# amazon-science/instruct-video-to-video

Measured on AMD Instinct MI355X. Metric: denoised video-frames/sec (16f@256x384, 50 DDIM steps), higher is better.
Workload: dtype fp16; 1 GPU; C2: 1 clip/step = VAE-encode + 50 DDIM steps (3-way CFG, text 7.5 / video 1.5) + VAE-decode, 16 frames @ 256x384, random-init full-width UNet+VAE; 5 independent clips in flight per GPU (stacked into every UNet launch, B = 3 x clips); frames=16, height=256, width=384, ddim_steps=50, clips_per_gpu=5, parallelism=clip-parallel x1, one all_gather, hip_graph=True, cfg_branch_streams=False, concurrent_clips=5, clip_mode=stacked, driver_mode=False, full=False

## Files before the change

### instruct-video-to-video_amd/csrc/winograd.hip

```cpp
#include "common.h"

namespace {

template <bool UP> __device__ __forceinline__ int lds_px(int sp) { return UP ? sp : sp ^ ((sp >> 1) & 1); }

template <bool NORM, bool UP>
__global__ __launch_bounds__(256) void wino_input_kernel(const half_t* __restrict__ x, const half_t* __restrict__ x2, const float* __restrict__ ab,
                                                         half_t* __restrict__ V, int64_t ldx, int64_t ldx2, int C1, int C, int NB, int H, int W,
                                                         int ipb, int images_per_sample, int silu, int64_t group_rows, int band_tr) {
    extern __shared__ __attribute__((aligned(16))) char smem[];
    const int tid = threadIdx.x, chunk = tid & 7, item0 = tid >> 3;
    const int nb0 = (int)blockIdx.x * ipb, c0 = (int)blockIdx.y * 64;
    const int trows = UP ? H : (H + 1) >> 1;
    const int tr0 = (int)blockIdx.z * band_tr, tr1 = min(tr0 + band_tr, trows);
    const bool whole = band_tr >= trows;
    const int row0 = whole ? 0 : (UP ? tr0 - 1 : 2 * tr0 - 1);
    const int nrows = whole ? H : (UP ? (tr1 - tr0) + 2 : 2 * (tr1 - tr0) + 2);
    const int HW = H * W, SW = nrows * W;
    const int SWs = UP ? SW : (SW + 1) & ~1;
    const bool second = x2 != nullptr && c0 >= C1;
    const half_t* src = second ? x2 + (c0 - C1) + chunk * 8 : x + c0 + chunk * 8;
    const int64_t ld = second ? ldx2 : ldx;
    const int nimg = min(ipb, NB - nb0);
    for (int it = item0; it < nimg * SW; it += 32) {
        const int img = it / SW, sp = it - img * SW;
        const int iy = row0 + sp / W;
        if ((unsigned)iy >= (unsigned)H) continue;
        half8 v = *(const half8*)(src + ((int64_t)(nb0 + img) * HW + sp + row0 * W) * ld);
        if (NORM) {
            const float* p = ab + ((int64_t)((nb0 + img) / images_per_sample) * C + c0 + chunk * 8) * 2;
            const float4 p0 = *(const float4*)p, p1 = *(const float4*)(p + 4), p2 = *(const float4*)(p + 8), p3 = *(const float4*)(p + 12);
            const float sc[8] = {p0.x, p0.z, p1.x, p1.z, p2.x, p2.z, p3.x, p3.z}, sh[8] = {p0.y, p0.w, p1.y, p1.w, p2.y, p2.w, p3.y, p3.w};
#pragma unroll
            for (int e = 0; e < 8; ++e) {
                float f = fmaf((float)v[e], sc[e], sh[e]);
                if (silu) f = silu_f(f);
                v[e] = (half_t)f;
            }
        }
        *(half8*)(smem + ((int64_t)img * SWs + lds_px<UP>(sp)) * 128 + chunk * 16) = v;
    }
    __syncthreads();
    if constexpr (UP) {
        const int bt = (tr1 - tr0) * W;
        for (int it = item0; it < nimg * bt; it += 32) {
            const int img = it / bt, tb_ = it - img * bt;
            const int y = tr0 + tb_ / W, xx = tb_ - (tb_ / W) * W;
            const int t = y * W + xx;
            const char* base = smem + (int64_t)img * SWs * 128 + chunk * 16;
            float hz[3][3][8];
#pragma unroll
            for (int r = 0; r < 3; ++r) {
                const int iy = y - 1 + r;
                float d[3][8];
#pragma unroll
                for (int c = 0; c < 3; ++c) {
                    const int ix = xx - 1 + c;
                    const bool ok = (unsigned)iy < (unsigned)H && (unsigned)ix < (unsigned)W;
                    half8 v = {0, 0, 0, 0, 0, 0, 0, 0};
                    if (ok) v = *(const half8*)(base + lds_px<UP>((iy - row0) * W + ix) * 128);
#pragma unroll
                    for (int e = 0; e < 8; ++e) d[c][e] = (float)v[e];
                }
#pragma unroll
                for (int e = 0; e < 8; ++e) {
                    hz[r][0][e] = d[0][e] - d[1][e];
                    hz[r][1][e] = 2.f * d[1][e];
                    hz[r][2][e] = d[1][e] - d[2][e];
                }
            }
            const int64_t trow = (int64_t)(nb0 + img) * HW + t;
            half_t* dst = V + trow * C + c0 + chunk * 8;
#pragma unroll
            for (int j = 0; j < 3; ++j) {
                half8 o[3];
#pragma unroll
                for (int e = 0; e < 8; ++e) {
                    o[0][e] = (half_t)(hz[0][j][e] - hz[1][j][e]);
                    o[1][e] = (half_t)(2.f * hz[1][j][e]);
                    o[2][e] = (half_t)(hz[1][j][e] - hz[2][j][e]);
                }
#pragma unroll
                for (int i = 0; i < 3; ++i) *(half8*)(dst + (int64_t)(i * 3 + j) * group_rows * C) = o[i];
            }
        }
        return;
    }
    const int th = (H + 1) >> 1, tw = (W + 1) >> 1, ntile = th * tw;
    const int bt = (tr1 - tr0) * tw;
    for (int it = item0; it < nimg * bt; it += 32) {
        const int img = it / bt, tb_ = it - img * bt;
        const int ty = tr0 + tb_ / tw, tx = tb_ - (tb_ / tw) * tw;
        const int t = ty * tw + tx;
        const char* base = smem + (int64_t)img * SWs * 128 + chunk * 16;
        float hz[4][4][8];
#pragma unroll
        for (int r = 0; r < 4; ++r) {
            const int iy = 2 * ty - 1 + r;
            float d[4][8];
#pragma unroll
            for (int c = 0; c < 4; ++c) {
                const int ix = 2 * tx - 1 + c;
                const bool ok = (unsigned)iy < (unsigned)H && (unsigned)ix < (unsigned)W;
                half8 v = {0, 0, 0, 0, 0, 0, 0, 0};
                if (ok) v = *(const half8*)(base + lds_px<UP>((iy - row0) * W + ix) * 128);
#pragma unroll
                for (int e = 0; e < 8; ++e) d[c][e] = (float)v[e];
            }
#pragma unroll
            for (int e = 0; e < 8; ++e) {
                hz[r][0][e] = d[0][e] - d[2][e];
                hz[r][1][e] = d[1][e] + d[2][e];
                hz[r][2][e] = d[2][e] - d[1][e];
                hz[r][3][e] = d[1][e] - d[3][e];
            }
        }
        const int64_t trow = (int64_t)(nb0 + img) * ntile + t;
        half_t* dst = V + trow * C + c0 + chunk * 8;
#pragma unroll
        for (int j = 0; j < 4; ++j) {
            half8 o[4];
#pragma unroll
            for (int e = 0; e < 8; ++e) {
                o[0][e] = (half_t)(hz[0][j][e] - hz[2][j][e]);
                o[1][e] = (half_t)(hz[1][j][e] + hz[2][j][e]);
                o[2][e] = (half_t)(hz[2][j][e] - hz[1][j][e]);
                o[3][e] = (half_t)(hz[1][j][e] - hz[3][j][e]);
            }
#pragma unroll
            for (int i = 0; i < 4; ++i) *(half8*)(dst + (int64_t)(i * 4 + j) * group_rows * C) = o[i];
        }
    }
}

template <bool RES, bool RB, bool UP>
__global__ __launch_bounds__(256) void wino_output_kernel(const half_t* __restrict__ Mo, const float* __restrict__ bias, const float* __restrict__ row_bias,
                                                          const half_t* __restrict__ res, half_t* __restrict__ y, int64_t group_rows, int64_t ntiles_total,
                                                          int Cout, int H, int W, int64_t ld_rb, int rows_per_group, int64_t ldr, int64_t ldy) {
    const int c8 = Cout >> 3;
    const int64_t idx = (int64_t)blockIdx.x * 256 + threadIdx.x;
    const int64_t tile = idx / c8;
    if (tile >= ntiles_total) return;
    const int ch = (int)(idx - tile * c8) * 8;
    const int th = UP ? H : (H + 1) >> 1, tw = UP ? W : (W + 1) >> 1, ntile = th * tw;
    const int OW = UP ? 2 * W : W, OH = UP ? 2 * H : H;
    const int nb = (int)(tile / ntile), t = (int)(tile - (int64_t)nb * ntile);
    const int ty = t / tw, tx = t - ty * tw;
    const half_t* src = Mo + tile * Cout + ch;
    float s[2][4][8];
    if constexpr (UP) {
#pragma unroll
        for (int j = 0; j < 3; ++j) {
            half8 m[3];
#pragma unroll
            for (int i = 0; i < 3; ++i) m[i] = *(const half8*)(src + (int64_t)(i * 3 + j) * group_rows * Cout);
            const int jj = j == 2 ? 3 : j;
#pragma unroll
            for (int e = 0; e < 8; ++e) {
                s[0][jj][e] = (float)m[0][e] + (float)m[1][e];
                s[1][jj][e] = (float)m[1][e] - (float)m[2][e];
            }
        }
#pragma unroll
        for (int e = 0; e < 8; ++e) s[0][2][e] = s[1][2][e] = 0.f;
    } else {
#pragma unroll
        for (int j = 0; j < 4; ++j) {
            half8 m[4];
#pragma unroll
            for (int i = 0; i < 4; ++i) m[i] = *(const half8*)(src + (int64_t)(i * 4 + j) * group_rows * Cout);
#pragma unroll
            for (int e = 0; e < 8; ++e) {
                s[0][j][e] = (float)m[0][e] + (float)m[1][e] + (float)m[2][e];
                s[1][j][e] = (float)m[1][e] - (float)m[2][e] - (float)m[3][e];
            }
        }
    }
    float b[8];
    {
        const float4 b0 = bias ? *(const float4*)(bias + ch) : make_float4(0.f, 0.f, 0.f, 0.f), b1 = bias ? *(const float4*)(bias + ch + 4) : make_float4(0.f, 0.f, 0.f, 0.f);
        b[0] = b0.x; b[1] = b0.y; b[2] = b0.z; b[3] = b0.w; b[4] = b1.x; b[5] = b1.y; b[6] = b1.z; b[7] = b1.w;
    }
    const int64_t m00 = ((int64_t)nb * OH + 2 * ty) * OW + 2 * tx;
    if (RB) {
        const float* rb = row_bias + (m00 / rows_per_group) * ld_rb + ch;
        const float4 r0 = *(const float4*)rb, r1 = *(const float4*)(rb + 4);
        b[0] += r0.x; b[1] += r0.y; b[2] += r0.z; b[3] += r0.w; b[4] += r1.x; b[5] += r1.y; b[6] += r1.z; b[7] += r1.w;
    }
#pragma unroll
    for (int i = 0; i < 2; ++i)
#pragma unroll
        for (int jj = 0; jj < 2; ++jj) {
            if (!UP && (2 * ty + i >= OH || 2 * tx + jj >= OW)) continue;
            const int64_t m = m00 + (int64_t)i * OW + jj;
            float v[8];
#pragma unroll
            for (int e = 0; e < 8; ++e)
                v[e] = (jj == 0 ? s[i][0][e] + s[i][1][e] + s[i][2][e] : s[i][1][e] - s[i][2][e] - s[i][3][e]) + b[e];
            if (RES) {
                const half8 r = *(const half8*)(res + m * ldr + ch);
#pragma unroll
                for (int e = 0; e < 8; ++e) v[e] += (float)r[e];
            }
            half8 o;
#pragma unroll
            for (int e = 0; e < 8; ++e) o[e] = (half_t)v[e];
            *(half8*)(y + m * ldy + ch) = o;
        }
}

}

extern "C" int insv2v_winograd_input(const insv2v_winograd_in_desc* dp, insv2v_stream_t stream) {
    if (!dp) return INSV2V_EINVAL;
    const insv2v_winograd_in_desc& d = *dp;
    if (!d.x || !d.v || d.NB <= 0 || d.H <= 0 || d.W <= 0 || d.C <= 0) return INSV2V_EINVAL;
    if ((d.C % 64) || (d.x2 && (d.C1 <= 0 || d.C1 >= d.C || (d.C1 % 64)))) return INSV2V_EUNSUPPORTED;
    if ((d.ldx & 7) || ((uintptr_t)d.x & 15) || ((uintptr_t)d.v & 15) || (d.x2 && ((d.ldx2 & 7) || ((uintptr_t)d.x2 & 15)))) return INSV2V_EINVAL;
    if (d.gn_ab && (d.gn_images_per_sample <= 0 || ((uintptr_t)d.gn_ab & 15))) return INSV2V_EINVAL;
    const int HW = d.H * d.W, ntile = d.upsample ? HW : ((d.H + 1) / 2) * ((d.W + 1) / 2);
    const int HWs = d.upsample ? HW : (HW + 1) & ~1;
    const int64_t tiles = (int64_t)d.NB * ntile;
    if (d.v_group_rows < tiles) return INSV2V_EINVAL;
    const int trows = d.upsample ? d.H : (d.H + 1) / 2;
    int band_tr = trows, ipb = 1;
    if (HWs * 128 <= 64 * 1024) {
        ipb = 32 / ntile;
        if (ipb < 1) ipb = 1;
        while (ipb > 1 && ipb * HWs * 128 > 64 * 1024) --ipb;
    } else {
        const int max_rows = 64 * 1024 / (d.W * 128);
        band_tr = d.upsample ? max_rows - 2 : (max_rows - 2) / 2;
        if (band_tr < 1) return INSV2V_EUNSUPPORTED;
    }
    const int nbands = (trows + band_tr - 1) / band_tr;
    const int srows = nbands == 1 ? d.H : (d.upsample ? band_tr + 2 : 2 * band_tr + 2);
    const dim3 grid((unsigned)((d.NB + ipb - 1) / ipb), (unsigned)(d.C / 64), (unsigned)nbands);
    const int slots = srows * d.W;
    const size_t lds = (size_t)ipb * (d.upsample ? slots : (slots + 1) & ~1) * 128;
#define WINO_IN(NORM, UP)                                                                                                                             \
    hipLaunchKernelGGL((wino_input_kernel<NORM, UP>), grid, dim3(256), lds, as_stream(stream), (const half_t*)d.x, (const half_t*)d.x2, d.gn_ab, (half_t*)d.v, \
                       d.ldx, d.ldx2, d.x2 ? d.C1 : d.C, d.C, d.NB, d.H, d.W, ipb, d.gn_ab ? d.gn_images_per_sample : 1, d.gn_ab ? d.gn_silu : 0, d.v_group_rows, band_tr)
    if (d.gn_ab) { if (d.upsample) WINO_IN(true, true); else WINO_IN(true, false); }
    else { if (d.upsample) WINO_IN(false, true); else WINO_IN(false, false); }
#undef WINO_IN
    return launch_status();
}

extern "C" int insv2v_winograd_output(const insv2v_winograd_out_desc* dp, insv2v_stream_t stream) {
    if (!dp) return INSV2V_EINVAL;
    const insv2v_winograd_out_desc& d = *dp;
    if (!d.m || !d.y || d.NB <= 0 || d.H <= 0 || d.W <= 0 || d.Cout <= 0) return INSV2V_EINVAL;
    if (d.Cout & 7) return INSV2V_EUNSUPPORTED;
    if ((d.ldy & 7) || ((uintptr_t)d.m & 15) || ((uintptr_t)d.y & 15) || (d.residual && ((d.ldr & 7) || ((uintptr_t)d.residual & 15)))) return INSV2V_EINVAL;
    if ((d.bias && ((uintptr_t)d.bias & 15)) || (d.row_bias && (((uintptr_t)d.row_bias & 15) || (d.ld_rb & 3) || d.rows_per_group <= 0 || d.rows_per_group % (d.H * d.W * (d.upsample ? 4 : 1)))))
        return INSV2V_EINVAL;
    const int64_t tiles = d.upsample ? (int64_t)d.NB * d.H * d.W : (int64_t)d.NB * ((d.H + 1) / 2) * ((d.W + 1) / 2);
    if (d.m_group_rows < tiles) return INSV2V_EINVAL;
    const int64_t n = tiles * (d.Cout / 8);
    const dim3 grid((unsigned)((n + 255) / 256));
#define WINO_OUT(RES, RB, UP)                                                                                                                        \
    hipLaunchKernelGGL((wino_output_kernel<RES, RB, UP>), grid, dim3(256), 0, as_stream(stream), (const half_t*)d.m, d.bias, d.row_bias, (const half_t*)d.residual, \
                       (half_t*)d.y, d.m_group_rows, tiles, d.Cout, d.H, d.W, d.ld_rb, d.rows_per_group, d.ldr, d.ldy)
    if (d.upsample) {
        if (d.residual) { if (d.row_bias) WINO_OUT(true, true, true); else WINO_OUT(true, false, true); }
        else { if (d.row_bias) WINO_OUT(false, true, true); else WINO_OUT(false, false, true); }
    } else {
        if (d.residual) { if (d.row_bias) WINO_OUT(true, true, false); else WINO_OUT(true, false, false); }
        else { if (d.row_bias) WINO_OUT(false, true, false); else WINO_OUT(false, false, false); }
    }
#undef WINO_OUT
    return launch_status();
}
```

Before: 15.77 frames/s.

## Rework Winograd input transform: wider channel slices, batched loads, flat grid, streaming stores

The Winograd input-transform kernel now optionally handles 128-channel slices per workgroup and issues four independent global loads per thread before normalizing, which raises memory-level parallelism. It also lowers the LDS target so more workgroups fit per CU, flattens the 3D grid into 1D, writes V with nontemporal stores, and computes the 4x4 transform one column at a time to cut register pressure. The aim is to make the bandwidth-bound transform that feeds the conv GEMMs cheaper. In exchange it adds template variants, clamped out-of-bounds loads, and more complex banding logic, and the 128-wide path drops the LDS swizzle, which may cause bank conflicts.

Result: no change. 15.76 frames/s (-0.0%).

```diff
diff --git a/instruct-video-to-video_amd/csrc/winograd.hip b/instruct-video-to-video_amd/csrc/winograd.hip
--- a/instruct-video-to-video_amd/csrc/winograd.hip
+++ b/instruct-video-to-video_amd/csrc/winograd.hip
@@ -1,66 +1,93 @@
 #include "common.h"
+#include <algorithm>
 
 namespace {
 
-template <bool UP> __device__ __forceinline__ int lds_px(int sp) { return UP ? sp : sp ^ ((sp >> 1) & 1); }
-
-template <bool NORM, bool UP>
+constexpr int kLoads = 4;
+constexpr int kWideSlice = 128;
+constexpr int kLdsWide = 40 * 1024;
+constexpr int kLdsNarrow = 32 * 1024;
+constexpr int kLdsMax = 64 * 1024;
+
+template <bool UP, int CS> __device__ __forceinline__ int lds_px(int sp) { return (UP || CS > 64) ? sp : sp ^ ((sp >> 1) & 1); }
+
+__device__ __forceinline__ void store_v(half_t* p, half8 o) { __builtin_nontemporal_store(o, (half8*)p); }
+
+template <bool NORM, bool UP, int CS>
 __global__ __launch_bounds__(256) void wino_input_kernel(const half_t* __restrict__ x, const half_t* __restrict__ x2, const float* __restrict__ ab,
                                                          half_t* __restrict__ V, int64_t ldx, int64_t ldx2, int C1, int C, int NB, int H, int W,
-                                                         int ipb, int images_per_sample, int silu, int64_t group_rows, int band_tr) {
+                                                         int ipb, int nslice, int nbands, int images_per_sample, int silu, int64_t group_rows, int band_tr) {
     extern __shared__ __attribute__((aligned(16))) char smem[];
-    const int tid = threadIdx.x, chunk = tid & 7, item0 = tid >> 3;
-    const int nb0 = (int)blockIdx.x * ipb, c0 = (int)blockIdx.y * 64;
+    constexpr int CPP = CS / 8, IPP = 256 / CPP, SLOT = CS * 2;
+    const int tid = threadIdx.x, chunk = tid % CPP, item0 = tid / CPP;
+    const int slice = (int)blockIdx.x % nslice, gb = (int)blockIdx.x / nslice, grp = gb / nbands, band = gb - grp * nbands;
+    const int nb0 = grp * ipb, c0 = slice * CS, c = c0 + chunk * 8;
+    const bool active = c < C;
     const int trows = UP ? H : (H + 1) >> 1;
-    const int tr0 = (int)blockIdx.z * band_tr, tr1 = min(tr0 + band_tr, trows);
+    const int tr0 = band * band_tr, tr1 = min(tr0 + band_tr, trows);
     const bool whole = band_tr >= trows;
     const int row0 = whole ? 0 : (UP ? tr0 - 1 : 2 * tr0 - 1);
     const int nrows = whole ? H : (UP ? (tr1 - tr0) + 2 : 2 * (tr1 - tr0) + 2);
     const int HW = H * W, SW = nrows * W;
     const int SWs = UP ? SW : (SW + 1) & ~1;
-    const bool second = x2 != nullptr && c0 >= C1;
-    const half_t* src = second ? x2 + (c0 - C1) + chunk * 8 : x + c0 + chunk * 8;
+    const int cl = active ? c : c0;
+    const bool second = x2 != nullptr && cl >= C1;
+    const half_t* src = second ? x2 + (cl - C1) : x + cl;
     const int64_t ld = second ? ldx2 : ldx;
     const int nimg = min(ipb, NB - nb0);
-    for (int it = item0; it < nimg * SW; it += 32) {
-        const int img = it / SW, sp = it - img * SW;
-        const int iy = row0 + sp / W;
-        if ((unsigned)iy >= (unsigned)H) continue;
-        half8 v = *(const half8*)(src + ((int64_t)(nb0 + img) * HW + sp + row0 * W) * ld);
-        if (NORM) {
-            const float* p = ab + ((int64_t)((nb0 + img) / images_per_sample) * C + c0 + chunk * 8) * 2;
-            const float4 p0 = *(const float4*)p, p1 = *(const float4*)(p + 4), p2 = *(const float4*)(p + 8), p3 = *(const float4*)(p + 12);
-            const float sc[8] = {p0.x, p0.z, p1.x, p1.z, p2.x, p2.z, p3.x, p3.z}, sh[8] = {p0.y, p0.w, p1.y, p1.w, p2.y, p2.w, p3.y, p3.w};
-#pragma unroll
-            for (int e = 0; e < 8; ++e) {
-                float f = fmaf((float)v[e], sc[e], sh[e]);
-                if (silu) f = silu_f(f);
-                v[e] = (half_t)f;
-            }
-        }
-        *(half8*)(smem + ((int64_t)img * SWs + lds_px<UP>(sp)) * 128 + chunk * 16) = v;
+    const int total = nimg * SW;
+    for (int it0 = item0; it0 < total; it0 += kLoads * IPP) {
+        half8 v[kLoads];
+        int slot[kLoads], im[kLoads];
+#pragma unroll
+        for (int u = 0; u < kLoads; ++u) {
+            const int it = it0 + u * IPP, itc = min(it, total - 1);
+            const int img = itc / SW, sp = itc - img * SW;
+            const int iy = row0 + sp / W, ix = sp - (sp / W) * W;
+            const int iyc = min(max(iy, 0), H - 1);
+            im[u] = nb0 + img;
+            slot[u] = (active && it < total && iy == iyc) ? img * SWs + lds_px<UP, CS>(sp) : -1;
+            v[u] = *(const half8*)(src + ((int64_t)im[u] * HW + iyc * W + ix) * ld);
+        }
+#pragma unroll
+        for (int u = 0; u < kLoads; ++u) {
+            if (slot[u] < 0) continue;
+            if (NORM) {
+                const float* p = ab + ((int64_t)(im[u] / images_per_sample) * C + c) * 2;
+                const float4 p0 = *(const float4*)p, p1 = *(const float4*)(p + 4), p2 = *(const float4*)(p + 8), p3 = *(const float4*)(p + 12);
+                const float sc[8] = {p0.x, p0.z, p1.x, p1.z, p2.x, p2.z, p3.x, p3.z}, sh[8] = {p0.y, p0.w, p1.y, p1.w, p2.y, p2.w, p3.y, p3.w};
+#pragma unroll
+                for (int e = 0; e < 8; ++e) {
+                    float f = fmaf((float)v[u][e], sc[e], sh[e]);
+                    if (silu) f = silu_f(f);
+                    v[u][e] = (half_t)f;
+                }
+            }
+            *(half8*)(smem + (int64_t)slot[u] * SLOT + chunk * 16) = v[u];
+        }
     }
     __syncthreads();
+    if (!active) return;
     if constexpr (UP) {
         const int bt = (tr1 - tr0) * W;
-        for (int it = item0; it < nimg * bt; it += 32) {
+        for (int it = item0; it < nimg * bt; it += IPP) {
             const int img = it / bt, tb_ = it - img * bt;
             const int y = tr0 + tb_ / W, xx = tb_ - (tb_ / W) * W;
             const int t = y * W + xx;
-            const char* base = smem + (int64_t)img * SWs * 128 + chunk * 16;
+            const char* base = smem + (int64_t)img * SWs * SLOT + chunk * 16;
             float hz[3][3][8];
 #pragma unroll
             for (int r = 0; r < 3; ++r) {
                 const int iy = y - 1 + r;
                 float d[3][8];
 #pragma unroll
-                for (int c = 0; c < 3; ++c) {
-                    const int ix = xx - 1 + c;
+                for (int cc = 0; cc < 3; ++cc) {
+                    const int ix = xx - 1 + cc;
                     const bool ok = (unsigned)iy < (unsigned)H && (unsigned)ix < (unsigned)W;
                     half8 v = {0, 0, 0, 0, 0, 0, 0, 0};
-                    if (ok) v = *(const half8*)(base + lds_px<UP>((iy - row0) * W + ix) * 128);
-#pragma unroll
-                    for (int e = 0; e < 8; ++e) d[c][e] = (float)v[e];
+                    if (ok) v = *(const half8*)(base + lds_px<UP, CS>((iy - row0) * W + ix) * SLOT);
+#pragma unroll
+                    for (int e = 0; e < 8; ++e) d[cc][e] = (float)v[e];
                 }
 #pragma unroll
                 for (int e = 0; e < 8; ++e) {
@@ -70,7 +97,7 @@
                 }
             }
             const int64_t trow = (int64_t)(nb0 + img) * HW + t;
-            half_t* dst = V + trow * C + c0 + chunk * 8;
+            half_t* dst = V + trow * C + c;
 #pragma unroll
             for (int j = 0; j < 3; ++j) {
                 half8 o[3];
@@ -81,54 +108,46 @@
                     o[2][e] = (half_t)(hz[1][j][e] - hz[2][j][e]);
                 }
 #pragma unroll
-                for (int i = 0; i < 3; ++i) *(half8*)(dst + (int64_t)(i * 3 + j) * group_rows * C) = o[i];
+                for (int i = 0; i < 3; ++i) store_v(dst + (int64_t)(i * 3 + j) * group_rows * C, o[i]);
             }
         }
         return;
     }
     const int th = (H + 1) >> 1, tw = (W + 1) >> 1, ntile = th * tw;
     const int bt = (tr1 - tr0) * tw;
-    for (int it = item0; it < nimg * bt; it += 32) {
+    for (int it = item0; it < nimg * bt; it += IPP) {
         const int img = it / bt, tb_ = it - img * bt;
         const int ty = tr0 + tb_ / tw, tx = tb_ - (tb_ / tw) * tw;
         const int t = ty * tw + tx;
-        const char* base = smem + (int64_t)img * SWs * 128 + chunk * 16;
-        float hz[4][4][8];
-#pragma unroll
-        for (int r = 0; r < 4; ++r) {
-            const int iy = 2 * ty - 1 + r;
-            float d[4][8];
-#pragma unroll
-            for (int c = 0; c < 4; ++c) {
-                const int ix = 2 * tx - 1 + c;
-                const bool ok = (unsigned)iy < (unsigned)H && (unsigned)ix < (unsigned)W;
-                half8 v = {0, 0, 0, 0, 0, 0, 0, 0};
-                if (ok) v = *(const half8*)(base + lds_px<UP>((iy - row0) * W + ix) * 128);
-#pragma unroll
-                for (int e = 0; e < 8; ++e) d[c][e] = (float)v[e];
-            }
+        const char* base = smem + (int64_t)img * SWs * SLOT + chunk * 16;
+        const int64_t trow = (int64_t)(nb0 + img) * ntile + t;
+        half_t* dst = V + trow * C + c;
+#pragma unroll 1
+        for (int j = 0; j < 4; ++j) {
+            const int ca = j == 0 ? 0 : (j == 2 ? 2 : 1), cb = j == 3 ? 3 : (j == 2 ? 1 : 2);
+            const int ixa = 2 * tx - 1 + ca, ixb = 2 * tx - 1 + cb;
+            const bool oka = (unsigned)ixa < (unsigned)W, okb = (unsigned)ixb < (unsigned)W;
+            float hz[4][8];
+#pragma unroll
+            for (int r = 0; r < 4; ++r) {
+                const int iy = 2 * ty - 1 + r;
+                const bool rok = (unsigned)iy < (unsigned)H;
+                half8 va = {0, 0, 0, 0, 0, 0, 0, 0}, vb = {0, 0, 0, 0, 0, 0, 0, 0};
+                if (rok && oka) va = *(const half8*)(base + lds_px<UP, CS>((iy - row0) * W + ixa) * SLOT);
+                if (rok && okb) vb = *(const half8*)(base + lds_px<UP, CS>((iy - row0) * W + ixb) * SLOT);
+#pragma unroll
+                for (int e = 0; e < 8; ++e) hz[r][e] = j == 1 ? (float)va[e] + (float)vb[e] : (float)va[e] - (float)vb[e];
+            }
+            half8 o[4];
 #pragma unroll
             for (int e = 0; e < 8; ++e) {
-                hz[r][0][e] = d[0][e] - d[2][e];
-                hz[r][1][e] = d[1][e] + d[2][e];
-                hz[r][2][e] = d[2][e] - d[1][e];
-                hz[r][3][e] = d[1][e] - d[3][e];
-            }
-        }
-        const int64_t trow = (int64_t)(nb0 + img) * ntile + t;
-        half_t* dst = V + trow * C + c0 + chunk * 8;
-#pragma unroll
-        for (int j = 0; j < 4; ++j) {
-            half8 o[4];
-#pragma unroll
-            for (int e = 0; e < 8; ++e) {
-                o[0][e] = (half_t)(hz[0][j][e] - hz[2][j][e]);
-                o[1][e] = (half_t)(hz[1][j][e] + hz[2][j][e]);
-                o[2][e] = (half_t)(hz[2][j][e] - hz[1][j][e]);
-                o[3][e] = (half_t)(hz[1][j][e] - hz[3][j][e]);
-            }
-#pragma unroll
-            for (int i = 0; i < 4; ++i) *(half8*)(dst + (int64_t)(i * 4 + j) * group_rows * C) = o[i];
+                o[0][e] = (half_t)(hz[0][e] - hz[2][e]);
+                o[1][e] = (half_t)(hz[1][e] + hz[2][e]);
+                o[2][e] = (half_t)(hz[2][e] - hz[1][e]);
+                o[3][e] = (half_t)(hz[1][e] - hz[3][e]);
+            }
+#pragma unroll
+            for (int i = 0; i < 4; ++i) store_v(dst + (int64_t)(i * 4 + j) * group_rows * C, o[i]);
         }
     }
 }
@@ -223,26 +242,37 @@
     const int64_t tiles = (int64_t)d.NB * ntile;
     if (d.v_group_rows < tiles) return INSV2V_EINVAL;
     const int trows = d.upsample ? d.H : (d.H + 1) / 2;
+    const int min_rows = d.upsample ? 3 : 4;
+    const bool wide = d.C > 64 && (d.upsample ? min_rows * d.W * kWideSlice * 2 <= kLdsMax : HWs * kWideSlice * 2 <= kLdsWide);
+    const int cs = wide ? kWideSlice : 64, kLdsTarget = wide ? kLdsWide : kLdsNarrow;
+    const int slot = cs * 2, ipp = 256 / (cs / 8);
     int band_tr = trows, ipb = 1;
-    if (HWs * 128 <= 64 * 1024) {
-        ipb = 32 / ntile;
-        if (ipb < 1) ipb = 1;
-        while (ipb > 1 && ipb * HWs * 128 > 64 * 1024) --ipb;
+    if (HWs * slot <= kLdsTarget) {
+        ipb = std::min(kLdsTarget / (HWs * slot), (4 * ipp + ntile - 1) / ntile);
+        ipb = std::max(1, std::min(ipb, d.NB));
     } else {
-        const int max_rows = 64 * 1024 / (d.W * 128);
+        int max_rows = kLdsTarget / (d.W * slot);
+        if (max_rows < min_rows) max_rows = kLdsMax / (d.W * slot);
         band_tr = d.upsample ? max_rows - 2 : (max_rows - 2) / 2;
         if (band_tr < 1) return INSV2V_EUNSUPPORTED;
+        if (band_tr >= trows && HWs * slot > kLdsMax) band_tr = trows - 1;
+        if (band_tr < 1) return INSV2V_EUNSUPPORTED;
     }
     const int nbands = (trows + band_tr - 1) / band_tr;
     const int srows = nbands == 1 ? d.H : (d.upsample ? band_tr + 2 : 2 * band_tr + 2);
-    const dim3 grid((unsigned)((d.NB + ipb - 1) / ipb), (unsigned)(d.C / 64), (unsigned)nbands);
+    const int nslice = (d.C + cs - 1) / cs;
+    const int64_t nwg = (int64_t)((d.NB + ipb - 1) / ipb) * nbands * nslice;
+    if (nwg > 0x7fffffff) return INSV2V_EUNSUPPORTED;
+    const dim3 grid((unsigned)nwg);
     const int slots = srows * d.W;
-    const size_t lds = (size_t)ipb * (d.upsample ? slots : (slots + 1) & ~1) * 128;
-#define WINO_IN(NORM, UP)                                                                                                                             \
-    hipLaunchKernelGGL((wino_input_kernel<NORM, UP>), grid, dim3(256), lds, as_stream(stream), (const half_t*)d.x, (const half_t*)d.x2, d.gn_ab, (half_t*)d.v, \
-                       d.ldx, d.ldx2, d.x2 ? d.C1 : d.C, d.C, d.NB, d.H, d.W, ipb, d.gn_ab ? d.gn_images_per_sample : 1, d.gn_ab ? d.gn_silu : 0, d.v_group_rows, band_tr)
-    if (d.gn_ab) { if (d.upsample) WINO_IN(true, true); else WINO_IN(true, false); }
-    else { if (d.upsample) WINO_IN(false, true); else WINO_IN(false, false); }
+    const size_t lds = (size_t)ipb * (d.upsample ? slots : (slots + 1) & ~1) * slot;
+#define WINO_IN(NORM, UP, CS)                                                                                                                         \
+    hipLaunchKernelGGL((wino_input_kernel<NORM, UP, CS>), grid, dim3(256), lds, as_stream(stream), (const half_t*)d.x, (const half_t*)d.x2, d.gn_ab, (half_t*)d.v, \
+                       d.ldx, d.ldx2, d.x2 ? d.C1 : d.C, d.C, d.NB, d.H, d.W, ipb, nslice, nbands, d.gn_ab ? d.gn_images_per_sample : 1, d.gn_ab ? d.gn_silu : 0, d.v_group_rows, band_tr)
+#define WINO_IN_CS(NORM, UP) do { if (cs == 64) WINO_IN(NORM, UP, 64); else WINO_IN(NORM, UP, kWideSlice); } while (0)
+    if (d.gn_ab) { if (d.upsample) WINO_IN_CS(true, true); else WINO_IN_CS(true, false); }
+    else { if (d.upsample) WINO_IN_CS(false, true); else WINO_IN_CS(false, false); }
+#undef WINO_IN_CS
 #undef WINO_IN
     return launch_status();
 }
```
